# menschj/PGW4ERA5

Hardware: NVIDIA B200
Metric: global 0.25deg ERA5 timesteps/s (higher is better)
Workload: dtype f32 storage; f64 geopotential/ps iteration

## Files before the change

pgw4era5_b200/csrc/pgw_column.cuh:

```cuda
#pragma once
#include <cuda.h>
#include <limits.h>

#include "pgw_common.cuh"

namespace pgw {

constexpr int kColumnThreads = 128;
#ifndef PGW_NODE_L2_AHEAD
#define PGW_NODE_L2_AHEAD 2
#endif
constexpr int kL2Ahead = PGW_NODE_L2_AHEAD;

struct Pair2 { float lo, hi; };
__device__ __forceinline__ Pair2 load_pair(const pgw_tslab &s, uint32_t off) {
    Pair2 r;
    r.lo = __ldg(s.lo + off);
    r.hi = __ldg(s.hi + off);
    return r;
}
__device__ __forceinline__ double blend_f64(const pgw_tslab &s, const Pair2 &v) {
    const double lo = (double)v.lo;
    if (s.x_new == 0.0) return lo;
    return ((double)v.hi - lo) / s.x_hi * s.x_new + lo;
// ... 222 lines not shown
}
__device__ __forceinline__ void tma_prefetch_2d(const CUtensorMap *map, int c0, int c1) {
    asm volatile("cp.async.bulk.prefetch.tensor.2d.L2.global [%0, {%1, %2}];"
                 ::"l"(reinterpret_cast<uint64_t>(map)), "r"(c0), "r"(c1) : "memory");
}
__device__ __forceinline__ void tma_commit() { asm volatile("cp.async.bulk.commit_group;" ::: "memory"); }
template <int N>
__device__ __forceinline__ void tma_wait_read() { asm volatile("cp.async.bulk.wait_group.read %0;" ::"n"(N) : "memory"); }
__device__ __forceinline__ void tma_wait_all() { asm volatile("cp.async.bulk.wait_group 0;" ::: "memory"); }

}

struct pgw_column_plan {
    bool ref;
    bool tma;
    int lst, np;
    size_t smem;
    bool fast;
    bool local;
    int ncand;
    bool reinterp;
};
bool pgw_tma_eligible(const pgw_timestep_args *a, int lst_generic, int *lst_tma, size_t *smem);
int pgw_launch_column_tma(const pgw_timestep_args *a, const pgw_column_plan &plan, cudaStream_t st);
int pgw_ensure_smem(const void *kernel, int slot, size_t smem, int np);
```

pgw4era5_b200/csrc/pgw_column_tma.cu:

```cuda
#include "pgw_column.cuh"

#include <stdlib.h>
#include <string.h>

namespace pgw {

#ifndef PGW_X2
#define PGW_X2 1
#endif
#ifndef PGW_UNIFORM_TOP
#define PGW_UNIFORM_TOP 0
#endif
#ifndef PGW_TMA_SLOTS
#define PGW_TMA_SLOTS 4
#endif
constexpr int kTmaSlots = PGW_TMA_SLOTS;
#ifndef PGW_TMA_L2_AHEAD
#define PGW_TMA_L2_AHEAD 0
#endif
constexpr int kTmaL2Ahead = PGW_TMA_L2_AHEAD;
#ifndef PGW_TMA_UNROLL_PARKED
#define PGW_TMA_UNROLL_PARKED 1
#endif
#ifndef PGW_TMA_UNROLL_STREAMED
#define PGW_TMA_UNROLL_STREAMED 1
#endif
constexpr int kUnrollParked = PGW_TMA_UNROLL_PARKED, kUnrollStreamed = PGW_TMA_UNROLL_STREAMED;
constexpr double kTaylorMaxRel = 0.012;
constexpr int kTmaMaxLev = 160;

struct TmaParams {
    CUtensorMap in[4];
    CUtensorMap out[4];
    float2 m[kTmaMaxLev];
};

struct F4 { float x, y, z, w; };
struct TagParked { static constexpr bool value = true; };
struct TagStreamed { static constexpr bool value = false; };
__device__ __forceinline__ F4 ldg4(const float4 *p) { const float4 v = __ldg(p); return F4{v.x, v.y, v.z, v.w}; }

template <bool FAST, int NLEV_C, int NP_C>
__global__ void __launch_bounds__(kColumnThreads + 32, 3)
pgw_column_tma_kernel(const __grid_constant__ pgw_timestep_args a, const __grid_constant__ TmaParams tp,
                      const int lst_arg, const int np_arg) {
    constexpr int NT = kColumnThreads;
    extern __shared__ __align__(1024) unsigned char smem[];
    const int L = NLEV_C ? NLEV_C : a.nlev, K = a.nplev;
    const int np = NP_C ? NP_C : np_arg;
    const int lst = NLEV_C ? NLEV_C - NP_C : lst_arg;
    float *const ring = reinterpret_cast<float *>(smem);
    float2 *const st_Te = reinterpret_cast<float2 *>(ring + kTmaSlots * 8 * NT);
    double2 *const hl0 = reinterpret_cast<double2 *>(st_Te + (size_t)np * NT);
    float2 *const m0p = reinterpret_cast<float2 *>(hl0 + (np + 1));
    float *const s_plev = reinterpret_cast<float *>(m0p + np);
    float *const s_inv_plev = s_plev + K;
    float *const s_inv_w = s_inv_plev + K;
#if PGW_UNIFORM_TOP
    const int K3 = 3 * K + ((3 * K) & 1), Lp = L + (L & 1);
    float *const s_ut = s_plev + K3;
    int *const s_un = reinterpret_cast<int *>(s_ut + Lp);
    uint64_t *const bar_full = reinterpret_cast<uint64_t *>(s_un + Lp);
#else
    uint64_t *const bar_full = reinterpret_cast<uint64_t *>(s_plev + 3 * K + ((3 * K) & 1));
#endif
    uint64_t *const bar_done = bar_full + kTmaSlots;
    const double2 *const s_hl = hl0 - lst;
    const float2 *const s_m = m0p - lst;

    const int tid = threadIdx.x;
    for (int i = tid; i <= np; i += NT + 32) hl0[i] = make_double2(a.ak[lst + i], a.bk[lst + i]);
    for (int i = tid; i < np; i += NT + 32) m0p[i] = make_float2((float)a.akm[lst + i], (float)a.bkm[lst + i]);
    for (int i = tid; i < K; i += NT + 32) {
        const int f0 = a.plev_descending ? (K - 1 - i) : i;
        const float p0 = (float)a.plev[f0];
        s_plev[i] = p0;
        s_inv_plev[i] = 1.0f / p0;
        if (i + 1 < K) {
            const float p1 = (float)a.plev[a.plev_descending ? (K - 2 - i) : (i + 1)];
            s_inv_w[i] = 1.0f / log2f(p1 / p0);
        } else s_inv_w[i] = 0.0f;
    }
    if (tid == 0) {
        for (int i = 0; i < kTmaSlots; ++i) { mbar_init(bar_full + i, 1); mbar_init(bar_done + i, NT); }
        asm volatile("fence.mbarrier_init.release.cluster;" ::: "memory");
    }
    __syncthreads();
#if PGW_UNIFORM_TOP
    for (int l = tid; l < L; l += NT + 32) {
        const float2 m = tp.m[l];
        int nd = -1;
        for (int k = K - 1; k >= 0; --k)
            if (s_plev[k] <= m.x) { nd = k; break; }
        s_un[l] = nd;
        s_ut[l] = nd >= 0 ? fast_lg2(m.x * s_inv_plev[nd]) * s_inv_w[nd] : 0.0f;
    }
    __syncthreads();
#endif

    const uint32_t n = (uint32_t)a.ncol;
    const int npairs = (L + 1) >> 1, np1 = np >> 1;

    if (tid >= NT) {
        if (tid != NT) return;
        const int c0 = (int)(blockIdx.x * NT);
        auto pair_row = [&](int j) { const int r = L - 2 - 2 * j; return r < 0 ? 0 : r; };
        auto load_pair_slot = [&](int j) {
            const int s = j % kTmaSlots;
            float *dst = ring + s * 8 * NT;
            mbar_arrive_expect_tx(bar_full + s, 4u * 2u * NT * sizeof(float));
#pragma unroll
            for (int v = 0; v < 4; ++v) tma_load_2d(dst + v * 2 * NT, &tp.in[v], c0, pair_row(j), bar_full + s);
        };
        auto l2_pair = [&](int j) {
            if (j < npairs) {
// ... 10 lines not shown
            mbar_wait_backoff(bar_done + s, (j / kTmaSlots) & 1);
            const int row = pair_row(j);
            tma_store_2d(&tp.out[0], c0, row, src);
            if (j >= np1) tma_store_2d(&tp.out[1], c0, row, src + 2 * NT);
            tma_store_2d(&tp.out[2], c0, row, src + 4 * NT);
            tma_store_2d(&tp.out[3], c0, row, src + 6 * NT);
            tma_commit();
            tma_wait_read<1>();
            if (j >= 1 && j - 1 + kTmaSlots < npairs) load_pair_slot(j - 1 + kTmaSlots);
            l2_pair(j + kTmaSlots + kTmaL2Ahead);
        }
        tma_wait_all();
        return;
    }

    const uint32_t c_raw = blockIdx.x * NT + tid;
    const uint32_t c = (c_raw >= n) ? n - 1 : c_raw;
    const bool valid = c_raw < n;
    unsigned errbits = 0;
    int k_pref = INT32_MAX, k_bound = INT32_MAX;

    const float ps_f = __ldg(a.PS + c);
    const Pair2 r_sic = load_pair(a.siconc, c), r_ts = load_pair(a.ts, c), r_tos = load_pair(a.tos, c);
    const Pair2 r_psh = load_pair(a.ps_hist, c), r_tas = load_pair(a.tas, c), r_hurs = load_pair(a.hurs, c);
    const Pair2 r_zg = load_pair(a.zg_ref, c);
    const float r_ice = __ldg(a.FR_SEA_ICE + c), r_land = __ldg(a.FR_LAND + c), r_skin = __ldg(a.T_SKIN + c);
    const float r_clim = __ldg(a.ts_clim + c), r_fis = __ldg(a.FIS + c);
    const double PSd = (double)ps_f;

    const float w_t = slab_weight(a.d4);
    const float4 *const d4lo = reinterpret_cast<const float4 *>(a.d4.lo);
    const float4 *const d4hi = reinterpret_cast<const float4 *>(a.d4.hi);
    const int desc = a.plev_descending;
    auto node_off = [&](int j) { return (uint32_t)(desc ? (K - 1 - j) : j) * n + c; };
    auto blend4 = [&](const F4 &x0, const F4 &x1) {
        return F4{blend_f32(w_t, x0.x, x1.x), blend_f32(w_t, x0.y, x1.y), blend_f32(w_t, x0.z, x1.z),
                  blend_f32(w_t, x0.w, x1.w)};
// ... 19 lines not shown
    if (s_node < 0) { errbits |= PGW_ERR_PS_HIST_RANGE; s_node = 0; }
    const float min_src_p0 = (s_node == 0) ? psh : s_plev[0];

    const int j_lo = w_lo < 0 ? 0 : w_lo, j_hi = (w_lo >= 0 && w_lo + 1 < K) ? w_lo + 1 : j_lo;
    const F4 rl0 = ldg4(d4lo + node_off(j_lo)), rl1 = ldg4(d4hi + node_off(j_lo));
    const F4 rh0 = ldg4(d4lo + node_off(j_hi)), rh1 = ldg4(d4hi + node_off(j_hi));
    const int j_s1 = s_node >= 1 ? s_node - 1 : 0;
    const F4 rs0 = ldg4(d4lo + node_off(j_s1)), rs1 = ldg4(d4hi + node_off(j_s1));
    F4 n0{0.f, 0.f, 0.f, 0.f}, n1 = n0, m0 = n0, m1 = n0;
    if (w_lo >= 1) { n0 = ldg4(d4lo + node_off(w_lo - 1)); n1 = ldg4(d4hi + node_off(w_lo - 1)); }
    if (w_lo >= 2) { m0 = ldg4(d4lo + node_off(w_lo - 2)); m1 = ldg4(d4hi + node_off(w_lo - 2)); }
#pragma unroll
    for (int d = 3; d <= kL2Ahead; ++d)
        if (w_lo - d >= 0) l2_node(w_lo - d);

    {
        float sic = (float)((double)r_ice + blend_f64(a.siconc, r_sic) / 100.0);
        sic = sic < 0.0f ? 0.0f : (sic > 1.0f ? 1.0f : sic);
        const double dts = blend_f64(a.ts, r_ts);
        const double dtos = blend_f64(a.tos, r_tos);
        double comb = dts;
        if (!isnan(sic) && !isnan(dtos)) {
            float fr = sic + r_land;
            fr = fr < 0.0f ? 0.0f : (fr > 1.0f ? 1.0f : fr);
            comb = (double)fr * dts + (double)(1.0f - fr) * dtos;
        }
        const double clim = (double)r_clim;
        if (valid) {
            a.FR_SEA_ICE_out[c] = sic;
            a.T_SKIN_out[c] = (float)((double)r_skin + comb);
        }
        for (int s = 0; s < a.nsoil; ++s) {
            const double dso = clim + a.soil_decay[s] * (comb - clim);
            const float so = (float)((double)__ldg(a.T_SO + (uint32_t)s * n + c) + dso);
            if (valid) a.T_SO_out[(uint32_t)s * n + c] = so;
        }
    }

    float w_p_lo, w_inv_p_lo, w_inv_w;
    F4 x_lo = blend4(rl0, rl1), x_d{0.f, 0.f, 0.f, 0.f};
    F4 nb = blend4(n0, n1);
    if (w_lo >= 0) {
        w_p_lo = s_plev[w_lo]; w_inv_p_lo = s_inv_plev[w_lo]; w_inv_w = s_inv_w[w_lo];
        if (w_lo + 1 < K) {
            const F4 x_hi = blend4(rh0, rh1);
            x_d = F4{x_hi.x - x_lo.x, x_hi.y - x_lo.y, x_hi.z - x_lo.z, x_hi.w - x_lo.w};
        }
    } else {
        w_p_lo = 0.0f; w_inv_p_lo = 1.0f; w_inv_w = 0.0f;
    }
    const float sfc_ta = (float)blend_f64(a.tas, r_tas), sfc_hur = (float)blend_f64(a.hurs, r_hurs);
    bool bot_on = true;
    float b_p1, b_inv_p1, b_inv_w, b_psh, b_ta1, b_hur1, b_dta, b_dhur;
    {
        const F4 xs = blend4(rs0, rs1);
        const bool has = s_node >= 1;
        b_p1 = has ? s_plev[j_s1] : 0.0f;
        b_inv_p1 = has ? s_inv_plev[j_s1] : 1.0f;
        b_psh = has ? psh : 0.0f;
        b_inv_w = has ? fast_rcp(fast_lg2(psh * b_inv_p1)) : 0.0f;
        b_ta1 = has ? xs.x : sfc_ta; b_hur1 = has ? xs.y : sfc_hur;
        b_dta = sfc_ta - b_ta1; b_dhur = sfc_hur - b_hur1;
    }

    struct Dlt { float ta, hur, ua, va; };
    const int32_t off_step = desc ? (int32_t)n : -(int32_t)n;
// ... 76 lines not shown
        return d;
    };
#endif
    auto sfc_override = [&](float p, Dlt &d) {
        if (bot_on) {
            if (p > b_p1) {
                const float tb = fast_lg2(p * b_inv_p1) * b_inv_w;
                const bool below = p >= b_psh;
                d.ta = below ? sfc_ta : fmaf(tb, b_dta, b_ta1);
                d.hur = below ? sfc_hur : fmaf(tb, b_dhur, b_hur1);
            } else bot_on = false;
        }
    };

    LnConst lk{2.0 / 3.0, 2.0 / 5.0, 2.0 / 7.0};
    asm volatile("" : "+d"(lk.c3), "+d"(lk.c5), "+d"(lk.c7));

    const double pref = a.p_ref;
    const double2 hl_sfc = s_hl[L];
    double pb_era = fma(PSd, hl_sfc.y, hl_sfc.x);
    double acc_era = 0.0;
    bool era_open = pb_era >= pref;
    if (!era_open) { errbits |= PGW_ERR_PREF_BELOW_SFC; k_pref = 0; }
    float psn_f = ps_f;

    double acc_res = 0.0, acc_T0 = 0.0, acc_part0 = 0.0, t_low_d = 0.0;
    double S1 = 0.0, S2 = 0.0, S3 = 0.0, S4 = 0.0;
    float H1 = 0.0f, H2 = 0.0f, H3 = 0.0f;
    int lstar = -1;
    auto rcp64 = [](double v) { double r = rcp64_approx(v); return fma(r, fma(-v, r, 1.0), r); };
    auto taylor_add = [&](int l, double Pb, double Pt, double tpd, float hq, float w, float dl, double sgn) {
        const double ub = s_hl[l + 1].y * rcp64(Pb), ut = s_hl[l].y * rcp64(Pt);
        const double d1 = ub - ut, sm = ub + ut, m2 = ub * ut;
        const double q2 = fma(sm, sm, -2.0 * m2);
        const double d2 = d1 * sm, d3 = d1 * (q2 + m2), d4 = d2 * q2;
        const double ts = sgn * tpd;
        S1 = fma(ts, d1, S1); S2 = fma(ts, d2, S2); S3 = fma(ts, d3, S3); S4 = fma(ts, d4, S4);
        const float D1 = (float)d1, D2 = -0.5f * (float)d2, D3 = (1.0f / 3.0f) * (float)d3;
        const float hs = (float)sgn * hq, w2 = w * w;
// ... 13 lines not shown
            const float hq_t = (0.61f * 0.622f) * e_pgw * g;
            const double tvp = fma(tpd, (double)hq_t, tpd);
            const double dl = ln_ratio<FAST>(pb_era, pt, lk);
            acc_era = fma(rtv, dl, acc_era);
            acc_res = fma((td + (double)dta) - tpd, dl, acc_res);
            if (era_open) {
                acc_T0 = fma(tvp, dl, acc_T0);
                taylor_add(l, pb_era, Pt, tpd, t_pgw * hq_t, bm * g, (float)dl, 1.0);
            } else {
                acc_part0 = tvp * dl;
            }
            pb_era = Pt;
        }
    };

    auto fixed_point = [&]() {
        const double fis = (double)r_fis;
        const double phi_era = fis + acc_era;
        const double gdzg = blend_f64(a.zg_ref, r_zg) * kG;
        const float2 *const bTe = st_Te + (size_t)(L - 1 - lst) * NT + tid;
        const double t_low = t_low_d;
        const bool no_star = lstar < 0;
        if (no_star) lstar = lst;
        const double acc_k0 = acc_T0 + acc_part0;
        const int ld_hi = min(lstar + 1, L - 1), ld_lo = max(lstar - 1, lst);
        if (lstar + 1 <= L - 1) {
            const int l = lstar + 1;
            const double2 ht = s_hl[l], hb = s_hl[l + 1];
            const float2 m = s_m[l];
            const float2 te = bTe[-(L - 1 - l) * NT];
// ... 61 lines not shown
                if (l >= lst && pb >= pref) acc = layer(l, *pTe, pref, acc);
            }
            const double phi_pgw = fis + kRd * acc;
            const double err = (phi_pgw - phi_era) - gdzg;
            adj = -a.adj_factor * psn / (kRd * t_low) * err;
            double ae = (isnan(err) || !valid) ? 0.0 : fabs(err);
            ae = warp_max(ae);
            if ((tid & 31) == 0 && ae > 0.0)
                atomicMax(reinterpret_cast<unsigned long long *>(a.maxerr + k),
                          (unsigned long long)__double_as_longlong(ae));
        }
        if (valid) {
            a.PS_out[c] = psn_f;
            a.dps_out[c] = (float)dps;
        }
        const float2 *pTe = bTe;
        uint32_t o2 = (uint32_t)(L - 1) * n + c;
        float *const oQ = a.QV_out;
        for (int l = L - 1; l >= lst; --l, pTe -= NT, o2 -= n) {
            const float qv = qv_from_e(pTe->y, psn_f, s_m[l]);
            if (valid) st_stream(oQ + o2, qv);
        }
    };

    float2 *pTe = st_Te + (size_t)(L - 1 - lst) * NT + tid;
    auto pair_body = [&](const int j, auto parked_c) {
        constexpr bool parked = decltype(parked_c)::value;
        const int l = max(L - 1 - 2 * j, 1);
        float2 mm0, mm1;
        if (parked) { mm0 = s_m[l]; mm1 = s_m[l - 1]; } else { mm0 = tp.m[l]; mm1 = tp.m[l - 1]; }
        float *const sl = ring + (j % kTmaSlots) * 8 * NT + tid;
        const bool ready = mbar_test(bar_full + (j % kTmaSlots), (j / kTmaSlots) & 1);
#if PGW_X2
        const float2 p01 = __ffma2_rn(make_float2(ps_f, ps_f), make_float2(mm0.y, mm1.y), make_float2(mm0.x, mm1.x));
        const float p0 = p01.x, p1 = p01.y;
#else
        const float p0 = fmaf(ps_f, mm0.y, mm0.x), p1 = fmaf(ps_f, mm1.y, mm1.x);
#endif
#if PGW_UNIFORM_TOP
        Dlt d0, d1;
        if (!parked && mm0.y == 0.0f && mm1.y == 0.0f) { d0 = walk_uniform(l); d1 = walk_uniform(l - 1); }
        else { d0 = walk(p0); d1 = walk(p1); }
#else
        Dlt d0 = walk(p0);
        Dlt d1 = walk(p1);
#endif
        if (stale) refresh();
        if (!ready) mbar_wait(bar_full + (j % kTmaSlots), (j / kTmaSlots) & 1);
        const float t0 = sl[NT], q0 = sl[3 * NT], u0 = sl[5 * NT], v0 = sl[7 * NT];
        const float t1 = sl[0], q1 = sl[2 * NT], u1 = sl[4 * NT], v1 = sl[6 * NT];
        if (__any_sync(0xffffffffu, bot_on)) { sfc_override(p0, d0); sfc_override(p1, d1); }
        const bool cold = __all_sync(0xffffffffu, is_cold(t0, d0.ta) && is_cold(t1, d1.ta));
#if PGW_X2
        const float2 e01 = thermo_e_pgw_x2(cold, make_float2(p0, p1), make_float2(t0, t1), make_float2(q0, q1),
                                           make_float2(d0.ta, d1.ta), make_float2(d0.hur, d1.hur));
        const float e0 = e01.x, e1 = e01.y;
#else
        const float e0 = thermo_e_pgw(cold, p0, t0, q0, d0.ta, d0.hur);
        const float e1 = thermo_e_pgw(cold, p1, t1, q1, d1.ta, d1.hur);
#endif
#if PGW_X2
        const float2 tp01 = __fadd2_rn(make_float2(t0, t1), make_float2(d0.ta, d1.ta));
        const float2 up01 = __fadd2_rn(make_float2(u0, u1), make_float2(d0.ua, d1.ua));
        const float2 vp01 = __fadd2_rn(make_float2(v0, v1), make_float2(d0.va, d1.va));
        const float tp0 = tp01.x, tp1 = tp01.y;
        sl[NT] = tp0; sl[5 * NT] = up01.x; sl[7 * NT] = vp01.x;
        sl[0] = tp1; sl[4 * NT] = up01.y; sl[6 * NT] = vp01.y;
#else
        const float tp0 = t0 + d0.ta, tp1 = t1 + d1.ta;
        sl[NT] = tp0; sl[5 * NT] = u0 + d0.ua; sl[7 * NT] = v0 + d0.va;
        sl[0] = tp1; sl[4 * NT] = u1 + d1.ua; sl[6 * NT] = v1 + d1.va;
#endif
        if (parked) {
            fence_proxy_async();
            mbar_arrive(bar_done + (j % kTmaSlots));
            pTe[0] = make_float2(tp0, e0);
            pTe[-NT] = make_float2(tp1, e1);
            pTe -= 2 * NT;
            if (j == 0) t_low_d = (double)t0 + (double)d0.ta;
            era_layer(l, p0, mm0.y, t0, q0, d0.ta, tp0, e0);
            era_layer(l - 1, p1, mm1.y, t1, q1, d1.ta, tp1, e1);
        } else {
#if PGW_X2
            const float2 pn = __ffma2_rn(make_float2(psn_f, psn_f), make_float2(mm0.y, mm1.y), make_float2(mm0.x, mm1.x));
            const float2 den = __ffma2_rn(make_float2(-0.378f, -0.378f), e01, pn);
            const float2 qv = __fmul2_rn(__fmul2_rn(make_float2(0.622f, 0.622f), e01),
                                         make_float2(fast_rcp(den.x), fast_rcp(den.y)));
            sl[3 * NT] = qv.x;
            sl[2 * NT] = qv.y;
#else
            sl[3 * NT] = qv_from_e(e0, psn_f, mm0);
            sl[2 * NT] = qv_from_e(e1, psn_f, mm1);
#endif
            fence_proxy_async();
            mbar_arrive(bar_done + (j % kTmaSlots));
        }
    };
#ifdef PGW_TMA_ONE_LOOP
#pragma unroll 1
    for (int j = 0; j <= npairs; ++j) {
        if (j == np1) fixed_point();
        if (j == npairs) break;
        if (j < np1) pair_body(j, TagParked{}); else pair_body(j, TagStreamed{});
    }
#else
#pragma unroll kUnrollParked
    for (int j = 0; j < np1; ++j) pair_body(j, TagParked{});
    fixed_point();
#pragma unroll kUnrollStreamed
    for (int j = np1; j < npairs; ++j) pair_body(j, TagStreamed{});
#endif

    const float2 m_top = tp.m[0];
    float p_top = fmaf(ps_f, m_top.y, m_top.x);
    p_top = warp_min(p_top);
    const float min_src_p = warp_min(min_src_p0);
    if ((tid & 31) == 0) {
        atomicMin(reinterpret_cast<unsigned *>(a.stats), __float_as_uint(fmaxf(p_top, 0.0f)));
        atomicMin(reinterpret_cast<unsigned *>(a.stats) + 1, __float_as_uint(fmaxf(min_src_p, 0.0f)));
    }
    if (errbits && valid) {
        atomicOr(a.err, errbits);
        if (a.first_k) {
            if (k_pref != INT32_MAX) atomicMin(a.first_k, k_pref);
            if (k_bound != INT32_MAX) atomicMin(a.first_k + 1, k_bound);
        }
    }
}

}

namespace {

using pgw::kColumnThreads;

size_t column_smem_tma(int nplev, int np, int nlev) {
    const int nt = kColumnThreads;
    size_t b = sizeof(float) * (size_t)pgw::kTmaSlots * 8 * nt +
               (size_t)np * nt * (2 * sizeof(float)) +
               sizeof(double) * 2 * (size_t)(np + 1) + sizeof(float) * 2 * (size_t)np;
    b += sizeof(float) * (size_t)(3 * nplev + ((3 * nplev) & 1));
#if PGW_UNIFORM_TOP
    b += 2 * sizeof(float) * (size_t)(nlev + (nlev & 1));
#endif
    b += sizeof(uint64_t) * 2 * pgw::kTmaSlots;
    return b;
}

typedef CUresult (*EncodeTiledFn)(CUtensorMap *, CUtensorMapDataType, cuuint32_t, void *, const cuuint64_t *,
                                  const cuuint64_t *, const cuuint32_t *, const cuuint32_t *,
                                  CUtensorMapInterleave, CUtensorMapSwizzle, CUtensorMapL2promotion,
                                  CUtensorMapFloatOOBfill);

EncodeTiledFn encode_tiled() {
    static EncodeTiledFn fn = []() -> EncodeTiledFn {
        void *p = nullptr;
        cudaDriverEntryPointQueryResult q;
        if (cudaGetDriverEntryPoint("cuTensorMapEncodeTiled", &p, cudaEnableDefault, &q) != cudaSuccess ||
            q != cudaDriverEntryPointSuccess)
            p = nullptr;
        cudaGetLastError();
// ... 28 lines not shown
    const cuuint64_t strides[1] = {(cuuint64_t)ncol * sizeof(float)};
    const cuuint32_t box[2] = {(cuuint32_t)kColumnThreads, 2u};
    const cuuint32_t estr[2] = {1u, 1u};
    CUresult r = encode_tiled()(m, CU_TENSOR_MAP_DATA_TYPE_FLOAT32, 2, const_cast<float *>(base), dims, strides, box,
                                estr, CU_TENSOR_MAP_INTERLEAVE_NONE, CU_TENSOR_MAP_SWIZZLE_NONE,
                                CU_TENSOR_MAP_L2_PROMOTION_L2_128B, CU_TENSOR_MAP_FLOAT_OOB_FILL_NONE);
    if (r != CUDA_SUCCESS) {
        pgw_set_error("cuTensorMapEncodeTiled failed (%d)", (int)r);
        return PGW_E_LAUNCH;
    }
    return PGW_OK;
}

}

bool pgw_tma_eligible(const pgw_timestep_args *a, int lst_generic, int *lst_tma, size_t *smem) {
    const int np = a->nlev - lst_generic;
    const int lst_even = lst_generic - (np & 1);
    if (!(a->akm_host && a->bkm_host) || lst_even < 0 || a->nlev > pgw::kTmaMaxLev || a->ncol % 4 != 0 ||
        a->ncol < kColumnThreads || a->ncol >= (1ll << 31))
        return false;
    const void *f[8] = {a->T, a->QV, a->U, a->V, a->T_out, a->QV_out, a->U_out, a->V_out};
    for (const void *p : f) if (!aligned16(p)) return false;
    if (!encode_tiled()) return false;
    *lst_tma = lst_even;
    *smem = column_smem_tma(a->nplev, a->nlev - lst_even, a->nlev);
    return true;
}

int pgw_launch_column_tma(const pgw_timestep_args *a, const pgw_column_plan &plan, cudaStream_t st) {
    int rc;
    pgw::TmaParams tp;
    const float *in[4] = {a->T, a->QV, a->U, a->V};
    float *out[4] = {a->T_out, a->QV_out, a->U_out, a->V_out};
    for (int v = 0; v < 4; ++v) {
        if ((rc = make_map(&tp.in[v], in[v], a->ncol, a->nlev)) != PGW_OK) return rc;
        if ((rc = make_map(&tp.out[v], out[v], a->ncol, a->nlev)) != PGW_OK) return rc;
    }
    for (int l = 0; l < pgw::kTmaMaxLev; ++l)
        tp.m[l] = l < a->nlev ? make_float2((float)a->akm_host[l], (float)a->bkm_host[l]) : make_float2(0.f, 0.f);
    const bool l137 = a->nlev == 137 && plan.np == 56 && plan.lst == 137 - 56;
    auto kern = plan.fast ? (l137 ? pgw::pgw_column_tma_kernel<true, 137, 56> : pgw::pgw_column_tma_kernel<true, 0, 0>)
                          : (l137 ? pgw::pgw_column_tma_kernel<false, 137, 56> : pgw::pgw_column_tma_kernel<false, 0, 0>);
    if ((rc = pgw_ensure_smem((const void *)kern, 4 + (plan.fast ? 1 : 0) + (l137 ? 2 : 0), plan.smem, plan.np)) != PGW_OK)
        return rc;
    const unsigned grid = (unsigned)((a->ncol + kColumnThreads - 1) / kColumnThreads);
    kern<<<grid, kColumnThreads + 32, plan.smem, st>>>(*a, tp, plan.lst, plan.np);
    return pgw_check_launch("pgw_column_tma_kernel");
}
```

pgw4era5_b200/csrc/pgw_misc.cu:

```cuda
#include <stdarg.h>
#include <stdio.h>

#include "pgw_common.cuh"

static thread_local char g_last_error[512] = "";

void pgw_set_error(const char *fmt, ...) {
    va_list ap;
    va_start(ap, fmt);
    vsnprintf(g_last_error, sizeof(g_last_error), fmt, ap);
    va_end(ap);
}

int pgw_check_launch(const char *what) {
    cudaError_t e = cudaGetLastError();
    if (e != cudaSuccess) {
        pgw_set_error("%s: %s", what, cudaGetErrorString(e));
        return PGW_E_LAUNCH;
    }
    return PGW_OK;
}

int pgw_ensure_smem(const void *kernel, int slot, size_t smem, int np) {
    constexpr int kMaxDev = 64, kSlots = 16;
    static thread_local size_t configured[kMaxDev][kSlots] = {};
    int dev = 0;
    if (cudaGetDevice(&dev) != cudaSuccess) return pgw_check_launch("cudaGetDevice");
    const bool cached = dev >= 0 && dev < kMaxDev && slot >= 0 && slot < kSlots;
    if (cached && smem <= configured[dev][slot]) return PGW_OK;
    int max_optin = 0;
    cudaDeviceGetAttribute(&max_optin, cudaDevAttrMaxSharedMemoryPerBlockOptin, dev);
    if (smem > (size_t)max_optin) {
        pgw_set_error("column stash needs %zu B of shared memory (%d levels below p_ref), device allows %d",
                      smem, np, max_optin);
        return PGW_E_SMEM;
    }
    if (cudaFuncSetAttribute(kernel, cudaFuncAttributeMaxDynamicSharedMemorySize, (int)smem) != cudaSuccess)
        return pgw_check_launch("cudaFuncSetAttribute");
    cudaFuncSetAttribute(kernel, cudaFuncAttributePreferredSharedMemoryCarveout, cudaSharedmemCarveoutMaxShared);
// ... 13 lines not shown
```

pgw4era5_b200/csrc/pgw_timestep.cu:

```cuda
#include "pgw_column.cuh"

#include <cuda_pipeline.h>
#include <stdlib.h>
#include <string.h>

namespace pgw {

struct Walk2 {
    int lo;
    float p_lo, inv_p_lo, inv_w;
    float a_lo, a_d, b_lo, b_d;
    float a_n0, a_n1, b_n0, b_n1;
    float a_m0, a_m1, b_m0, b_m1;
};

constexpr int kRing = 5;

template <int NT, bool FAST, bool REF, bool LOCAL = false, bool RI = false>
__global__ void __launch_bounds__(NT, REF ? 2 : 3)
pgw_column_kernel(const __grid_constant__ pgw_timestep_args a, const int lst, const int np, const int ncand,
                  const pgw_timestep_result *replay) {
    static_assert(!(REF && LOCAL), "PGW_FLAG_LOCAL_PREF runs with float64 accumulation only");
    static_assert(!(RI && (REF || LOCAL)), "PGW_FLAG_REINTERP runs with a scalar p_ref and float64 accumulation");
    int k_spec = a.k_spec;
// ... 828 lines not shown
                          a->dps_out, a->dps_traj, a->maxerr, a->stats, a->err};
    for (const void *p : need) if (!p) return PGW_E_INVALID;
    if ((reinterpret_cast<uintptr_t>(a->d4.lo) | reinterpret_cast<uintptr_t>(a->d4.hi)) & 15u) return PGW_E_INVALID;
    if (a->nsoil > 0 && (!a->T_SO || !a->T_SO_out)) return PGW_E_INVALID;
    if ((a->flags & PGW_FLAG_REINTERP) && (a->flags & (PGW_FLAG_LOCAL_PREF | PGW_FLAG_REF_DTYPES))) return PGW_E_INVALID;
    if (a->flags & PGW_FLAG_LOCAL_PREF) {
        if (a->flags & PGW_FLAG_REF_DTYPES) return PGW_E_INVALID;
        if (a->nzg < 1 || a->nzg > 64 || !(a->p_floor > 0.0)) return PGW_E_INVALID;
        if ((unsigned long long)a->ncol * (unsigned long long)a->nzg >= (1ull << 31)) return PGW_E_INVALID;
        if (!a->zg.lo || !a->zg.hi || !a->zg_plev || !a->zg_plev_host || !a->pref_traj || !a->p_ref_out)
            return PGW_E_INVALID;
    }
    return PGW_OK;
}

bool tma_allowed() {
    const char *e = getenv("PGW_COLUMN_PATH");
    return !(e && strcmp(e, "generic") == 0);
}

pgw_column_plan plan_column(const pgw_timestep_args *a) {
    pgw_column_plan p;
    p.local = (a->flags & PGW_FLAG_LOCAL_PREF) != 0;
    const double p_stash = p.local ? a->p_floor : a->p_ref;
    p.lst = stash_top(a->ak_host, a->bk_host, a->nlev, p_stash, a->ps_bound);
    p.np = a->nlev - p.lst;
    p.ref = (a->flags & PGW_FLAG_REF_DTYPES) != 0;
    p.reinterp = (a->flags & PGW_FLAG_REINTERP) != 0;
    p.smem = column_smem(a->nlev, a->nplev, p.np, kColumnThreads, p.ref);
    p.ncand = 0;
    if (p.local) {
        for (int i = 0; i < a->nzg; ++i) p.ncand += a->zg_plev_host[i] >= a->p_floor;
        p.smem += local_pref_smem(a->nzg, p.ncand, kColumnThreads);
    }
    p.tma = false;
    int lst_tma = 0;
    size_t smem_tma = 0;
    if (tma_allowed() &&
        !(a->flags & (PGW_FLAG_DIRECT | PGW_FLAG_REF_DTYPES | PGW_FLAG_LOCAL_PREF | PGW_FLAG_REINTERP)) &&
        pgw_tma_eligible(a, p.lst, &lst_tma, &smem_tma)) {
        p.tma = true;
        p.lst = lst_tma;
        p.np = a->nlev - lst_tma;
        p.smem = smem_tma;
    }
    p.fast = true;
    for (int l = p.lst; l < a->nlev; ++l)
        for (double ps : {p_stash, a->ps_bound}) {
            const double pt = a->ak_host[l] + ps * a->bk_host[l], pb = a->ak_host[l + 1] + ps * a->bk_host[l + 1];
            if (!(pt > 0.0) || !((pb - pt) / (pb + pt) < 0.055)) p.fast = false;
        }
    return p;
}

int launch_reinterp(const pgw_timestep_args *a, const pgw_column_plan &plan, const pgw_timestep_result *replay,
                    cudaStream_t st) {
    auto kern = plan.fast ? pgw::pgw_column_kernel<kColumnThreads, true, false, false, true>
                          : pgw::pgw_column_kernel<kColumnThreads, false, false, false, true>;
    int rc = pgw_ensure_smem((const void *)kern, plan.fast ? 11 : 10, plan.smem, plan.np);
// ... 108 lines not shown
```

Baseline: 817.9.

## Add warp-specialized persistent column kernel splitting parked and streamed phases

Adds a persistent kernel whose blocks hold one producer warpgroup, issuing TMA loads for two separate rings, and two consumer warpgroups. One consumer runs the parked phase (stash and fixed-point iteration), then hands per-column state through shared memory and mbarriers to the other, which runs the streamed phase. Producer and consumer register budgets are rebalanced with setmaxnreg. The aim is to overlap the serial fixed-point work of one tile with streaming the upper levels of the previous tile, at the cost of more shared memory, handoff traffic and tighter occupancy.

```diff
diff --git a/pgw4era5_b200/csrc/pgw_column.cuh b/pgw4era5_b200/csrc/pgw_column.cuh
--- a/pgw4era5_b200/csrc/pgw_column.cuh
+++ b/pgw4era5_b200/csrc/pgw_column.cuh
@@ -260,6 +260,7 @@
 struct pgw_column_plan {
     bool ref;
     bool tma;
+    bool ws;
     int lst, np;
     size_t smem;
     bool fast;
@@ -267,6 +268,6 @@
     int ncand;
     bool reinterp;
 };
-bool pgw_tma_eligible(const pgw_timestep_args *a, int lst_generic, int *lst_tma, size_t *smem);
+bool pgw_tma_eligible(const pgw_timestep_args *a, int lst_generic, int *lst_tma, size_t *smem, size_t *smem_ws);
 int pgw_launch_column_tma(const pgw_timestep_args *a, const pgw_column_plan &plan, cudaStream_t st);
 int pgw_ensure_smem(const void *kernel, int slot, size_t smem, int np);
diff --git a/pgw4era5_b200/csrc/pgw_column_tma.cu b/pgw4era5_b200/csrc/pgw_column_tma.cu
--- a/pgw4era5_b200/csrc/pgw_column_tma.cu
+++ b/pgw4era5_b200/csrc/pgw_column_tma.cu
@@ -28,6 +28,9 @@
 constexpr int kUnrollParked = PGW_TMA_UNROLL_PARKED, kUnrollStreamed = PGW_TMA_UNROLL_STREAMED;
 constexpr double kTaylorMaxRel = 0.012;
 constexpr int kTmaMaxLev = 160;
+#ifndef PGW_WS_CLOCKS
+#define PGW_WS_CLOCKS 0
+#endif
 
 struct TmaParams {
     CUtensorMap in[4];
@@ -39,6 +42,61 @@
 struct TagParked { static constexpr bool value = true; };
 struct TagStreamed { static constexpr bool value = false; };
 __device__ __forceinline__ F4 ldg4(const float4 *p) { const float4 v = __ldg(p); return F4{v.x, v.y, v.z, v.w}; }
+
+enum ColumnRole { kWhole, kParked, kStreamed };
+enum HandWord {
+    hPs, hPsn, hWlo, hOffM, hPlo, hInvPlo, hInvW, hXlo, hXd = hXlo + 4, hNb = hXd + 4, hM0 = hNb + 4,
+    hM1 = hM0 + 4, hBotOn = hM1 + 4, hBP1, hBInvP1, hBInvW, hBPsh, hBTa1, hBHur1, hBDta, hBDhur, hSfcTa, hSfcHur,
+    kHandWords
+};
+struct TileSmem {
+    float *ring;
+    uint64_t *bar_full, *bar_done;
+    float2 *st_Te;
+    const double2 *s_hl;
+    const float2 *s_m;
+    const float *s_plev, *s_inv_plev, *s_inv_w;
+    const float *s_ut;
+    const int *s_un;
+    float *hand;
+    uint64_t *hand_full, *hand_empty;
+    uint64_t *stash_free;
+};
+template <bool FAST, int NLEV_C, int NP_C, int ROLE>
+__device__ __forceinline__ void column_tile(const pgw_timestep_args &a, const TmaParams &tp, const TileSmem &sm,
+                                            int lst_arg, int np_arg, int tid, uint32_t tile, int qb, uint32_t hpar,
+                                            long long &wait_clk);
+
+__device__ __forceinline__ void fill_tables(const pgw_timestep_args &a, double2 *hl0, float2 *m0p, float *s_plev,
+                                            float *s_inv_plev, float *s_inv_w, int lst, int np, int K, int tid,
+                                            int stride) {
+    for (int i = tid; i <= np; i += stride) hl0[i] = make_double2(a.ak[lst + i], a.bk[lst + i]);
+    for (int i = tid; i < np; i += stride) m0p[i] = make_float2((float)a.akm[lst + i], (float)a.bkm[lst + i]);
+    for (int i = tid; i < K; i += stride) {
+        const int f0 = a.plev_descending ? (K - 1 - i) : i;
+        const float p0 = (float)a.plev[f0];
+        s_plev[i] = p0;
+        s_inv_plev[i] = 1.0f / p0;
+        if (i + 1 < K) {
+            const float p1 = (float)a.plev[a.plev_descending ? (K - 2 - i) : (i + 1)];
+            s_inv_w[i] = 1.0f / log2f(p1 / p0);
+        } else s_inv_w[i] = 0.0f;
+    }
+}
+#if PGW_UNIFORM_TOP
+__device__ __forceinline__ void fill_uniform(const TmaParams &tp, const float *s_plev, const float *s_inv_plev,
+                                             const float *s_inv_w, float *s_ut, int *s_un, int L, int K, int tid,
+                                             int stride) {
+    for (int l = tid; l < L; l += stride) {
+        const float2 m = tp.m[l];
+        int nd = -1;
+        for (int k = K - 1; k >= 0; --k)
+            if (s_plev[k] <= m.x) { nd = k; break; }
+        s_un[l] = nd;
+        s_ut[l] = nd >= 0 ? fast_lg2(m.x * s_inv_plev[nd]) * s_inv_w[nd] : 0.0f;
+    }
+}
+#endif
 
 template <bool FAST, int NLEV_C, int NP_C>
 __global__ void __launch_bounds__(kColumnThreads + 32, 3)
@@ -69,36 +127,17 @@
     const float2 *const s_m = m0p - lst;
 
     const int tid = threadIdx.x;
-    for (int i = tid; i <= np; i += NT + 32) hl0[i] = make_double2(a.ak[lst + i], a.bk[lst + i]);
-    for (int i = tid; i < np; i += NT + 32) m0p[i] = make_float2((float)a.akm[lst + i], (float)a.bkm[lst + i]);
-    for (int i = tid; i < K; i += NT + 32) {
-        const int f0 = a.plev_descending ? (K - 1 - i) : i;
-        const float p0 = (float)a.plev[f0];
-        s_plev[i] = p0;
-        s_inv_plev[i] = 1.0f / p0;
-        if (i + 1 < K) {
-            const float p1 = (float)a.plev[a.plev_descending ? (K - 2 - i) : (i + 1)];
-            s_inv_w[i] = 1.0f / log2f(p1 / p0);
-        } else s_inv_w[i] = 0.0f;
-    }
+    fill_tables(a, hl0, m0p, s_plev, s_inv_plev, s_inv_w, lst, np, K, tid, NT + 32);
     if (tid == 0) {
         for (int i = 0; i < kTmaSlots; ++i) { mbar_init(bar_full + i, 1); mbar_init(bar_done + i, NT); }
         asm volatile("fence.mbarrier_init.release.cluster;" ::: "memory");
     }
     __syncthreads();
 #if PGW_UNIFORM_TOP
-    for (int l = tid; l < L; l += NT + 32) {
-        const float2 m = tp.m[l];
-        int nd = -1;
-        for (int k = K - 1; k >= 0; --k)
-            if (s_plev[k] <= m.x) { nd = k; break; }
-        s_un[l] = nd;
-        s_ut[l] = nd >= 0 ? fast_lg2(m.x * s_inv_plev[nd]) * s_inv_w[nd] : 0.0f;
-    }
+    fill_uniform(tp, s_plev, s_inv_plev, s_inv_w, s_ut, s_un, L, K, tid, NT + 32);
     __syncthreads();
 #endif
 
-    const uint32_t n = (uint32_t)a.ncol;
     const int npairs = (L + 1) >> 1, np1 = np >> 1;
 
     if (tid >= NT) {
@@ -139,13 +178,60 @@
         return;
     }
 
-    const uint32_t c_raw = blockIdx.x * NT + tid;
+    long long no_clk = 0;
+    column_tile<FAST, NLEV_C, NP_C, kWhole>(
+        a, tp,
+        TileSmem{ring, bar_full, bar_done, st_Te, s_hl, s_m, s_plev, s_inv_plev, s_inv_w,
+#if PGW_UNIFORM_TOP
+                 s_ut, s_un,
+#else
+                 nullptr, nullptr,
+#endif
+                 nullptr, nullptr, nullptr, nullptr},
+        lst, np, tid, blockIdx.x, 0, 0, no_clk);
+}
+
+__device__ __forceinline__ void hand_wait(uint64_t *bar, uint32_t parity, long long &clk) {
+#if PGW_WS_CLOCKS
+    const long long t0 = clock64();
+    mbar_wait(bar, parity);
+    clk += clock64() - t0;
+#else
+    mbar_wait(bar, parity);
+#endif
+}
+
+template <bool FAST, int NLEV_C, int NP_C, int ROLE>
+__device__ __forceinline__ void column_tile(const pgw_timestep_args &a, const TmaParams &tp, const TileSmem &sm,
+                                            const int lst_arg, const int np_arg, const int tid, const uint32_t tile,
+                                            const int qb, const uint32_t hpar, long long &wait_clk) {
+    constexpr int NT = kColumnThreads;
+    constexpr bool kParkedPart = ROLE != kStreamed, kStreamedPart = ROLE != kParked;
+    const int L = NLEV_C ? NLEV_C : a.nlev, K = a.nplev;
+    const int np = NP_C ? NP_C : np_arg;
+    const int lst = NLEV_C ? NLEV_C - NP_C : lst_arg;
+    float *const ring = sm.ring;
+    uint64_t *const bar_full = sm.bar_full, *const bar_done = sm.bar_done;
+    float2 *const st_Te = sm.st_Te;
+    const double2 *const s_hl = sm.s_hl;
+    const float2 *const s_m = sm.s_m;
+    const float *const s_plev = sm.s_plev, *const s_inv_plev = sm.s_inv_plev, *const s_inv_w = sm.s_inv_w;
+#if PGW_UNIFORM_TOP
+    const float *const s_ut = sm.s_ut;
+    const int *const s_un = sm.s_un;
+#endif
+    const uint32_t n = (uint32_t)a.ncol;
+    const int npairs = (L + 1) >> 1, np1 = np >> 1;
+    float *const ho = sm.hand + tid;
+    if constexpr (ROLE == kStreamed) hand_wait(sm.hand_full, hpar, wait_clk);
+
+    const uint32_t c_raw = tile * NT + tid;
     const uint32_t c = (c_raw >= n) ? n - 1 : c_raw;
     const bool valid = c_raw < n;
     unsigned errbits = 0;
     int k_pref = INT32_MAX, k_bound = INT32_MAX;
 
-    const float ps_f = __ldg(a.PS + c);
+    const float ps_f = ROLE == kStreamed ? ho[hPs * NT] : __ldg(a.PS + c);
     const Pair2 r_sic = load_pair(a.siconc, c), r_ts = load_pair(a.ts, c), r_tos = load_pair(a.tos, c);
     const Pair2 r_psh = load_pair(a.ps_hist, c), r_tas = load_pair(a.tas, c), r_hurs = load_pair(a.hurs, c);
     const Pair2 r_zg = load_pair(a.zg_ref, c);
@@ -195,7 +281,7 @@
     for (int d = 3; d <= kL2Ahead; ++d)
         if (w_lo - d >= 0) l2_node(w_lo - d);
 
-    {
+    auto surface_update = [&]() {
         float sic = (float)((double)r_ice + blend_f64(a.siconc, r_sic) / 100.0);
         sic = sic < 0.0f ? 0.0f : (sic > 1.0f ? 1.0f : sic);
         const double dts = blend_f64(a.ts, r_ts);
@@ -216,7 +302,8 @@
             const float so = (float)((double)__ldg(a.T_SO + (uint32_t)s * n + c) + dso);
             if (valid) a.T_SO_out[(uint32_t)s * n + c] = so;
         }
-    }
+    };
+    if constexpr (ROLE != kParked) surface_update();
 
     float w_p_lo, w_inv_p_lo, w_inv_w;
     F4 x_lo = blend4(rl0, rl1), x_d{0.f, 0.f, 0.f, 0.f};
@@ -230,7 +317,7 @@
     } else {
         w_p_lo = 0.0f; w_inv_p_lo = 1.0f; w_inv_w = 0.0f;
     }
-    const float sfc_ta = (float)blend_f64(a.tas, r_tas), sfc_hur = (float)blend_f64(a.hurs, r_hurs);
+    float sfc_ta = (float)blend_f64(a.tas, r_tas), sfc_hur = (float)blend_f64(a.hurs, r_hurs);
     bool bot_on = true;
     float b_p1, b_inv_p1, b_inv_w, b_psh, b_ta1, b_hur1, b_dta, b_dhur;
     {
@@ -337,7 +424,7 @@
     };
 
     LnConst lk{2.0 / 3.0, 2.0 / 5.0, 2.0 / 7.0};
-    asm volatile("" : "+d"(lk.c3), "+d"(lk.c5), "+d"(lk.c7));
+    if constexpr (kParkedPart) asm volatile("" : "+d"(lk.c3), "+d"(lk.c5), "+d"(lk.c7));
 
     const double pref = a.p_ref;
     const double2 hl_sfc = s_hl[L];
@@ -346,6 +433,23 @@
     bool era_open = pb_era >= pref;
     if (!era_open) { errbits |= PGW_ERR_PREF_BELOW_SFC; k_pref = 0; }
     float psn_f = ps_f;
+
+    auto get4 = [&](int w) { return F4{ho[w * NT], ho[(w + 1) * NT], ho[(w + 2) * NT], ho[(w + 3) * NT]}; };
+    auto put4 = [&](int w, const F4 &v) {
+        ho[w * NT] = v.x; ho[(w + 1) * NT] = v.y; ho[(w + 2) * NT] = v.z; ho[(w + 3) * NT] = v.w;
+    };
+    if constexpr (ROLE == kStreamed) {
+        psn_f = ho[hPsn * NT];
+        w_lo = __float_as_int(ho[hWlo * NT]);
+        off_m = __float_as_uint(ho[hOffM * NT]);
+        w_p_lo = ho[hPlo * NT]; w_inv_p_lo = ho[hInvPlo * NT]; w_inv_w = ho[hInvW * NT];
+        x_lo = get4(hXlo); x_d = get4(hXd); nb = get4(hNb); m0 = get4(hM0); m1 = get4(hM1);
+        bot_on = __float_as_int(ho[hBotOn * NT]) != 0;
+        b_p1 = ho[hBP1 * NT]; b_inv_p1 = ho[hBInvP1 * NT]; b_inv_w = ho[hBInvW * NT]; b_psh = ho[hBPsh * NT];
+        b_ta1 = ho[hBTa1 * NT]; b_hur1 = ho[hBHur1 * NT]; b_dta = ho[hBDta * NT]; b_dhur = ho[hBDhur * NT];
+        sfc_ta = ho[hSfcTa * NT]; sfc_hur = ho[hSfcHur * NT];
+        mbar_arrive(sm.hand_empty);
+    }
 
     double acc_res = 0.0, acc_T0 = 0.0, acc_part0 = 0.0, t_low_d = 0.0;
     double S1 = 0.0, S2 = 0.0, S3 = 0.0, S4 = 0.0;
@@ -389,6 +493,15 @@
         }
     };
 
+    auto store_parked_qv = [&]() {
+        const float2 *pTe = st_Te + (size_t)(L - 1 - lst) * NT + tid;
+        uint32_t o2 = (uint32_t)(L - 1) * n + c;
+        float *const oQ = a.QV_out;
+        for (int l = L - 1; l >= lst; --l, pTe -= NT, o2 -= n) {
+            const float qv = qv_from_e(pTe->y, psn_f, s_m[l]);
+            if (valid) st_stream(oQ + o2, qv);
+        }
+    };
     auto fixed_point = [&]() {
         const double fis = (double)r_fis;
         const double phi_era = fis + acc_era;
@@ -480,13 +593,7 @@
             a.PS_out[c] = psn_f;
             a.dps_out[c] = (float)dps;
         }
-        const float2 *pTe = bTe;
-        uint32_t o2 = (uint32_t)(L - 1) * n + c;
-        float *const oQ = a.QV_out;
-        for (int l = L - 1; l >= lst; --l, pTe -= NT, o2 -= n) {
-            const float qv = qv_from_e(pTe->y, psn_f, s_m[l]);
-            if (valid) st_stream(oQ + o2, qv);
-        }
+        if constexpr (ROLE == kWhole) store_parked_qv();
     };
 
     float2 *pTe = st_Te + (size_t)(L - 1 - lst) * NT + tid;
@@ -495,8 +602,9 @@
         const int l = max(L - 1 - 2 * j, 1);
         float2 mm0, mm1;
         if (parked) { mm0 = s_m[l]; mm1 = s_m[l - 1]; } else { mm0 = tp.m[l]; mm1 = tp.m[l - 1]; }
-        float *const sl = ring + (j % kTmaSlots) * 8 * NT + tid;
-        const bool ready = mbar_test(bar_full + (j % kTmaSlots), (j / kTmaSlots) & 1);
+        const int q = qb + j;
+        float *const sl = ring + (q % kTmaSlots) * 8 * NT + tid;
+        const bool ready = mbar_test(bar_full + (q % kTmaSlots), (q / kTmaSlots) & 1);
 #if PGW_X2
         const float2 p01 = __ffma2_rn(make_float2(ps_f, ps_f), make_float2(mm0.y, mm1.y), make_float2(mm0.x, mm1.x));
         const float p0 = p01.x, p1 = p01.y;
@@ -512,7 +620,7 @@
         Dlt d1 = walk(p1);
 #endif
         if (stale) refresh();
-        if (!ready) mbar_wait(bar_full + (j % kTmaSlots), (j / kTmaSlots) & 1);
+        if (!ready) mbar_wait(bar_full + (q % kTmaSlots), (q / kTmaSlots) & 1);
         const float t0 = sl[NT], q0 = sl[3 * NT], u0 = sl[5 * NT], v0 = sl[7 * NT];
         const float t1 = sl[0], q1 = sl[2 * NT], u1 = sl[4 * NT], v1 = sl[6 * NT];
         if (__any_sync(0xffffffffu, bot_on)) { sfc_override(p0, d0); sfc_override(p1, d1); }
@@ -539,7 +647,7 @@
 #endif
         if (parked) {
             fence_proxy_async();
-            mbar_arrive(bar_done + (j % kTmaSlots));
+            mbar_arrive(bar_done + (q % kTmaSlots));
             pTe[0] = make_float2(tp0, e0);
             pTe[-NT] = make_float2(tp1, e1);
             pTe -= 2 * NT;
@@ -559,10 +667,11 @@
             sl[2 * NT] = qv_from_e(e1, psn_f, mm1);
 #endif
             fence_proxy_async();
-            mbar_arrive(bar_done + (j % kTmaSlots));
+            mbar_arrive(bar_done + (q % kTmaSlots));
         }
     };
 #ifdef PGW_TMA_ONE_LOOP
+    static_assert(ROLE == kWhole, "PGW_TMA_ONE_LOOP: the one-phase kernel only");
 #pragma unroll 1
     for (int j = 0; j <= npairs; ++j) {
         if (j == np1) fixed_point();
@@ -570,12 +679,22 @@
         if (j < np1) pair_body(j, TagParked{}); else pair_body(j, TagStreamed{});
     }
 #else
+    if constexpr (kParkedPart) {
+        if constexpr (ROLE == kParked) hand_wait(sm.stash_free, hpar ^ 1u, wait_clk);
 #pragma unroll kUnrollParked
-    for (int j = 0; j < np1; ++j) pair_body(j, TagParked{});
-    fixed_point();
+        for (int j = 0; j < np1; ++j) pair_body(j, TagParked{});
+        fixed_point();
+    }
+    if constexpr (kStreamedPart) {
+        if constexpr (ROLE == kStreamed) {
+            store_parked_qv();
+            mbar_arrive(sm.stash_free);
+        }
 #pragma unroll kUnrollStreamed
-    for (int j = np1; j < npairs; ++j) pair_body(j, TagStreamed{});
-#endif
+        for (int j = np1; j < npairs; ++j) pair_body(j, TagStreamed{});
+    }
+#endif
+    if constexpr (!kParkedPart) return;
 
     const float2 m_top = tp.m[0];
     float p_top = fmaf(ps_f, m_top.y, m_top.x);
@@ -592,6 +711,163 @@
             if (k_bound != INT32_MAX) atomicMin(a.first_k + 1, k_bound);
         }
     }
+
+    if constexpr (ROLE == kParked) {
+        hand_wait(sm.hand_empty, hpar ^ 1u, wait_clk);
+        ho[hPs * NT] = ps_f; ho[hPsn * NT] = psn_f;
+        ho[hWlo * NT] = __int_as_float(w_lo); ho[hOffM * NT] = __uint_as_float(off_m);
+        ho[hPlo * NT] = w_p_lo; ho[hInvPlo * NT] = w_inv_p_lo; ho[hInvW * NT] = w_inv_w;
+        put4(hXlo, x_lo); put4(hXd, x_d); put4(hNb, nb); put4(hM0, m0); put4(hM1, m1);
+        ho[hBotOn * NT] = __int_as_float(bot_on ? 1 : 0);
+        ho[hBP1 * NT] = b_p1; ho[hBInvP1 * NT] = b_inv_p1; ho[hBInvW * NT] = b_inv_w; ho[hBPsh * NT] = b_psh;
+        ho[hBTa1 * NT] = b_ta1; ho[hBHur1 * NT] = b_hur1; ho[hBDta * NT] = b_dta; ho[hBDhur * NT] = b_dhur;
+        ho[hSfcTa * NT] = sfc_ta; ho[hSfcHur * NT] = sfc_hur;
+        mbar_arrive(sm.hand_full);
+    }
+}
+
+#if PGW_WS_CLOCKS
+__device__ unsigned long long g_ws_clocks[4];
+#endif
+
+__device__ __forceinline__ void ws_producer(const TmaParams &tp, float *ring, uint64_t *bar_full, uint64_t *bar_done,
+                                            int L, int jb, int per, bool store_qv, uint32_t ntiles) {
+    constexpr int NT = kColumnThreads;
+    const int Q = (int)((ntiles - blockIdx.x + gridDim.x - 1) / gridDim.x) * per;
+    auto coords = [&](int q, int &c0, int &row) {
+        const int it = q / per, j = jb + (q - it * per);
+        c0 = (int)((blockIdx.x + (uint32_t)it * gridDim.x) * NT);
+        const int r = L - 2 - 2 * j;
+        row = r < 0 ? 0 : r;
+    };
+    auto load_pair_slot = [&](int q) {
+        int c0, row;
+        coords(q, c0, row);
+        const int s = q % kTmaSlots;
+        float *dst = ring + s * 8 * NT;
+        mbar_arrive_expect_tx(bar_full + s, 4u * 2u * NT * sizeof(float));
+#pragma unroll
+        for (int v = 0; v < 4; ++v) tma_load_2d(dst + v * 2 * NT, &tp.in[v], c0, row, bar_full + s);
+    };
+    for (int q = 0; q < kTmaSlots && q < Q; ++q) load_pair_slot(q);
+#pragma unroll 1
+    for (int q = 0; q < Q; ++q) {
+        const int s = q % kTmaSlots;
+        const float *src = ring + s * 8 * NT;
+        mbar_wait_backoff(bar_done + s, (q / kTmaSlots) & 1);
+        int c0, row;
+        coords(q, c0, row);
+        tma_store_2d(&tp.out[0], c0, row, src);
+        if (store_qv) tma_store_2d(&tp.out[1], c0, row, src + 2 * NT);
+        tma_store_2d(&tp.out[2], c0, row, src + 4 * NT);
+        tma_store_2d(&tp.out[3], c0, row, src + 6 * NT);
+        tma_commit();
+        tma_wait_read<1>();
+        if (q >= 1 && q - 1 + kTmaSlots < Q) load_pair_slot(q - 1 + kTmaSlots);
+    }
+    tma_wait_all();
+}
+
+template <bool FAST, int NLEV_C, int NP_C>
+__global__ void __launch_bounds__(3 * kColumnThreads, 2)
+pgw_column_ws_kernel(const __grid_constant__ pgw_timestep_args a, const __grid_constant__ TmaParams tp,
+                     const int lst_arg, const int np_arg) {
+    constexpr int NT = kColumnThreads, NTH = 3 * kColumnThreads;
+    extern __shared__ __align__(1024) unsigned char smem[];
+    const int L = NLEV_C ? NLEV_C : a.nlev, K = a.nplev;
+    const int np = NP_C ? NP_C : np_arg;
+    const int lst = NLEV_C ? NLEV_C - NP_C : lst_arg;
+    float *const ring_p = reinterpret_cast<float *>(smem);
+    float *const ring_s = ring_p + kTmaSlots * 8 * NT;
+    float2 *const st_Te = reinterpret_cast<float2 *>(ring_s + kTmaSlots * 8 * NT);
+    double2 *const hl0 = reinterpret_cast<double2 *>(st_Te + (size_t)np * NT);
+    float2 *const m0p = reinterpret_cast<float2 *>(hl0 + (np + 1));
+    float *const s_plev = reinterpret_cast<float *>(m0p + np);
+    float *const s_inv_plev = s_plev + K;
+    float *const s_inv_w = s_inv_plev + K;
+#if PGW_UNIFORM_TOP
+    const int K3 = 3 * K + ((3 * K) & 1), Lp = L + (L & 1);
+    float *const s_ut = s_plev + K3;
+    int *const s_un = reinterpret_cast<int *>(s_ut + Lp);
+    float *const hand = reinterpret_cast<float *>(s_un + Lp);
+#else
+    float *const hand = s_plev + 3 * K + ((3 * K) & 1);
+#endif
+    uint64_t *const bar_full_p = reinterpret_cast<uint64_t *>(hand + kHandWords * NT);
+    uint64_t *const bar_done_p = bar_full_p + kTmaSlots;
+    uint64_t *const bar_full_s = bar_done_p + kTmaSlots;
+    uint64_t *const bar_done_s = bar_full_s + kTmaSlots;
+    uint64_t *const hand_full = bar_done_s + kTmaSlots, *const hand_empty = hand_full + 1;
+    uint64_t *const stash_free = hand_empty + 1;
+
+    const int tid = threadIdx.x;
+    fill_tables(a, hl0, m0p, s_plev, s_inv_plev, s_inv_w, lst, np, K, tid, NTH);
+    if (tid == 0) {
+        for (int i = 0; i < kTmaSlots; ++i) {
+            mbar_init(bar_full_p + i, 1); mbar_init(bar_done_p + i, NT);
+            mbar_init(bar_full_s + i, 1); mbar_init(bar_done_s + i, NT);
+        }
+        mbar_init(hand_full, NT);
+        mbar_init(hand_empty, NT);
+        mbar_init(stash_free, NT);
+        asm volatile("fence.mbarrier_init.release.cluster;" ::: "memory");
+    }
+    __syncthreads();
+#if PGW_UNIFORM_TOP
+    fill_uniform(tp, s_plev, s_inv_plev, s_inv_w, s_ut, s_un, L, K, tid, NTH);
+    __syncthreads();
+#endif
+
+    const uint32_t ntiles = (uint32_t)((a.ncol + NT - 1) / NT);
+    const int npairs = (L + 1) >> 1, np1 = np >> 1, ns = npairs - np1;
+    const int wg = tid / NT;
+    if (wg == 0) {
+        asm volatile("setmaxnreg.dec.sync.aligned.u32 24;" ::: "memory");
+        if ((tid & 31) != 0 || tid >= 64) return;
+        if (tid == 0) ws_producer(tp, ring_p, bar_full_p, bar_done_p, L, 0, np1, false, ntiles);
+        else ws_producer(tp, ring_s, bar_full_s, bar_done_s, L, np1, ns, true, ntiles);
+        return;
+    }
+    long long wait_clk = 0;
+#if PGW_WS_CLOCKS
+    const long long t_start = clock64();
+#endif
+    if (wg == 1) {
+        asm volatile("setmaxnreg.inc.sync.aligned.u32 128;" ::: "memory");
+        const TileSmem sm{ring_p, bar_full_p, bar_done_p, st_Te, hl0 - lst, m0p - lst, s_plev, s_inv_plev, s_inv_w,
+#if PGW_UNIFORM_TOP
+                          s_ut, s_un,
+#else
+                          nullptr, nullptr,
+#endif
+                          hand, hand_full, hand_empty, stash_free};
+        uint32_t it = 0;
+#pragma unroll 1
+        for (uint32_t t = blockIdx.x; t < ntiles; t += gridDim.x, ++it)
+            column_tile<FAST, NLEV_C, NP_C, kParked>(a, tp, sm, lst, np, tid - NT, t, (int)it * np1, it & 1u, wait_clk);
+    } else {
+        asm volatile("setmaxnreg.inc.sync.aligned.u32 88;" ::: "memory");
+        const TileSmem sm{ring_s, bar_full_s, bar_done_s, st_Te, hl0 - lst, m0p - lst, s_plev, s_inv_plev, s_inv_w,
+#if PGW_UNIFORM_TOP
+                          s_ut, s_un,
+#else
+                          nullptr, nullptr,
+#endif
+                          hand, hand_full, hand_empty, stash_free};
+        uint32_t it = 0;
+#pragma unroll 1
+        for (uint32_t t = blockIdx.x; t < ntiles; t += gridDim.x, ++it)
+            column_tile<FAST, NLEV_C, NP_C, kStreamed>(a, tp, sm, lst, np, tid - 2 * NT, t, (int)it * ns - np1, it & 1u,
+                                                       wait_clk);
+    }
+#if PGW_WS_CLOCKS
+    if ((tid & 31) == 0) {
+        atomicAdd(&g_ws_clocks[wg - 1], (unsigned long long)wait_clk);
+        atomicAdd(&g_ws_clocks[wg + 1], (unsigned long long)(clock64() - t_start));
+    }
+#else
+    (void)wait_clk;
+#endif
 }
 
 }
@@ -611,6 +887,24 @@
 #endif
     b += sizeof(uint64_t) * 2 * pgw::kTmaSlots;
     return b;
+}
+
+size_t column_smem_ws(int nplev, int np, int nlev) {
+    const int nt = kColumnThreads;
+    return column_smem_tma(nplev, np, nlev) + sizeof(float) * (size_t)pgw::kTmaSlots * 8 * nt +
+           sizeof(float) * (size_t)pgw::kHandWords * nt + sizeof(uint64_t) * (2 * pgw::kTmaSlots + 3);
+}
+
+bool ws_fits(size_t smem) {
+    int dev = 0, per_sm = 0, optin = 0, reserved = 0;
+    if (cudaGetDevice(&dev) != cudaSuccess ||
+        cudaDeviceGetAttribute(&per_sm, cudaDevAttrMaxSharedMemoryPerMultiprocessor, dev) != cudaSuccess ||
+        cudaDeviceGetAttribute(&optin, cudaDevAttrMaxSharedMemoryPerBlockOptin, dev) != cudaSuccess ||
+        cudaDeviceGetAttribute(&reserved, cudaDevAttrReservedSharedMemoryPerBlock, dev) != cudaSuccess) {
+        cudaGetLastError();
+        return false;
+    }
+    return smem <= (size_t)optin && 2 * (smem + (size_t)reserved) <= (size_t)per_sm;
 }
 
 typedef CUresult (*EncodeTiledFn)(CUtensorMap *, CUtensorMapDataType, cuuint32_t, void *, const cuuint64_t *,
@@ -669,7 +963,7 @@
 
 }
 
-bool pgw_tma_eligible(const pgw_timestep_args *a, int lst_generic, int *lst_tma, size_t *smem) {
+bool pgw_tma_eligible(const pgw_timestep_args *a, int lst_generic, int *lst_tma, size_t *smem, size_t *smem_ws) {
     const int np = a->nlev - lst_generic;
     const int lst_even = lst_generic - (np & 1);
     if (!(a->akm_host && a->bkm_host) || lst_even < 0 || a->nlev > pgw::kTmaMaxLev || a->ncol % 4 != 0 ||
@@ -680,6 +974,8 @@
     if (!encode_tiled()) return false;
     *lst_tma = lst_even;
     *smem = column_smem_tma(a->nplev, a->nlev - lst_even, a->nlev);
+    const size_t ws = column_smem_ws(a->nplev, a->nlev - lst_even, a->nlev);
+    *smem_ws = ws_fits(ws) ? ws : 0;
     return true;
 }
 
@@ -695,6 +991,21 @@
     for (int l = 0; l < pgw::kTmaMaxLev; ++l)
         tp.m[l] = l < a->nlev ? make_float2((float)a->akm_host[l], (float)a->bkm_host[l]) : make_float2(0.f, 0.f);
     const bool l137 = a->nlev == 137 && plan.np == 56 && plan.lst == 137 - 56;
+    if (plan.ws) {
+        auto kern = plan.fast ? (l137 ? pgw::pgw_column_ws_kernel<true, 137, 56> : pgw::pgw_column_ws_kernel<true, 0, 0>)
+                              : (l137 ? pgw::pgw_column_ws_kernel<false, 137, 56> : pgw::pgw_column_ws_kernel<false, 0, 0>);
+        if ((rc = pgw_ensure_smem((const void *)kern, 16 + (plan.fast ? 1 : 0) + (l137 ? 2 : 0), plan.smem, plan.np)) !=
+            PGW_OK)
+            return rc;
+        int dev = 0, nsm = 0;
+        if (cudaGetDevice(&dev) != cudaSuccess ||
+            cudaDeviceGetAttribute(&nsm, cudaDevAttrMultiProcessorCount, dev) != cudaSuccess)
+            return pgw_check_launch("cudaDeviceGetAttribute");
+        const long long ntiles = (a->ncol + kColumnThreads - 1) / kColumnThreads;
+        const unsigned grid = (unsigned)(ntiles < 2ll * nsm ? ntiles : 2ll * nsm);
+        kern<<<grid, 3 * kColumnThreads, plan.smem, st>>>(*a, tp, plan.lst, plan.np);
+        return pgw_check_launch("pgw_column_ws_kernel");
+    }
     auto kern = plan.fast ? (l137 ? pgw::pgw_column_tma_kernel<true, 137, 56> : pgw::pgw_column_tma_kernel<true, 0, 0>)
                           : (l137 ? pgw::pgw_column_tma_kernel<false, 137, 56> : pgw::pgw_column_tma_kernel<false, 0, 0>);
     if ((rc = pgw_ensure_smem((const void *)kern, 4 + (plan.fast ? 1 : 0) + (l137 ? 2 : 0), plan.smem, plan.np)) != PGW_OK)
@@ -703,3 +1014,13 @@
     kern<<<grid, kColumnThreads + 32, plan.smem, st>>>(*a, tp, plan.lst, plan.np);
     return pgw_check_launch("pgw_column_tma_kernel");
 }
+
+#if PGW_WS_CLOCKS
+extern "C" int pgw_ws_clocks(unsigned long long *out4) {
+    if (cudaMemcpyFromSymbol(out4, pgw::g_ws_clocks, sizeof(pgw::g_ws_clocks)) != cudaSuccess)
+        return pgw_check_launch("pgw_ws_clocks");
+    static const unsigned long long zero[4] = {0, 0, 0, 0};
+    if (cudaMemcpyToSymbol(pgw::g_ws_clocks, zero, sizeof(zero)) != cudaSuccess) return pgw_check_launch("pgw_ws_clocks");
+    return PGW_OK;
+}
+#endif
diff --git a/pgw4era5_b200/csrc/pgw_misc.cu b/pgw4era5_b200/csrc/pgw_misc.cu
--- a/pgw4era5_b200/csrc/pgw_misc.cu
+++ b/pgw4era5_b200/csrc/pgw_misc.cu
@@ -22,7 +22,7 @@
 }
 
 int pgw_ensure_smem(const void *kernel, int slot, size_t smem, int np) {
-    constexpr int kMaxDev = 64, kSlots = 16;
+    constexpr int kMaxDev = 64, kSlots = 20;
     static thread_local size_t configured[kMaxDev][kSlots] = {};
     int dev = 0;
     if (cudaGetDevice(&dev) != cudaSuccess) return pgw_check_launch("cudaGetDevice");
diff --git a/pgw4era5_b200/csrc/pgw_timestep.cu b/pgw4era5_b200/csrc/pgw_timestep.cu
--- a/pgw4era5_b200/csrc/pgw_timestep.cu
+++ b/pgw4era5_b200/csrc/pgw_timestep.cu
@@ -866,9 +866,9 @@
     return PGW_OK;
 }
 
-bool tma_allowed() {
+bool column_path_is(const char *name) {
     const char *e = getenv("PGW_COLUMN_PATH");
-    return !(e && strcmp(e, "generic") == 0);
+    return e && strcmp(e, name) == 0;
 }
 
 pgw_column_plan plan_column(const pgw_timestep_args *a) {
@@ -885,16 +885,17 @@
         for (int i = 0; i < a->nzg; ++i) p.ncand += a->zg_plev_host[i] >= a->p_floor;
         p.smem += local_pref_smem(a->nzg, p.ncand, kColumnThreads);
     }
-    p.tma = false;
+    p.tma = p.ws = false;
     int lst_tma = 0;
-    size_t smem_tma = 0;
-    if (tma_allowed() &&
+    size_t smem_tma = 0, smem_ws = 0;
+    if (!column_path_is("generic") &&
         !(a->flags & (PGW_FLAG_DIRECT | PGW_FLAG_REF_DTYPES | PGW_FLAG_LOCAL_PREF | PGW_FLAG_REINTERP)) &&
-        pgw_tma_eligible(a, p.lst, &lst_tma, &smem_tma)) {
+        pgw_tma_eligible(a, p.lst, &lst_tma, &smem_tma, &smem_ws)) {
         p.tma = true;
+        p.ws = smem_ws != 0 && !column_path_is("tma_pairs");
         p.lst = lst_tma;
         p.np = a->nlev - lst_tma;
-        p.smem = smem_tma;
+        p.smem = p.ws ? smem_ws : smem_tma;
     }
     p.fast = true;
     for (int l = p.lst; l < a->nlev; ++l)
```

Result: no change. 823.2 (median of 6 runs) (+0.6%).
